# BICLab/Spike2Former

Measured on AMD Instinct MI355X. Metric: fwd+bwd images/sec, 512x512 T=4 ADE20K-150, higher is better.
Workload: dtype f32 (fp32-equivalent: bf16 hi+mid+lo split operands on bf16 MFMA, fp32 accumulate; spike maps stored as bf16, exact); 1 GPU; C2: 512x512 T=4 K=150 Meta-SpikeFormer [64, 128, 256, 360] + MaskFormer head, per-GPU batch 2; global_batch=2, parallelism=dp1, weights=random-init (name-seeded)

## Files before the change

spike2former_amd/csrc/pgemm.hip:

```cpp
#include "gemm_common.h"
#include <cstdlib>
#include <type_traits>

#pragma clang fp contract(fast)

namespace {

constexpr int PK = 32;
constexpr int PR = 64;
constexpr int PTERM = PR * PK;
constexpr int PBLOCK = 3 * PTERM;

typedef __attribute__((address_space(3))) void lds_void;
typedef const __attribute__((address_space(1))) void gbl_void;

__device__ __forceinline__ void dma16(const void* src, void* lds_dst) {
  __builtin_amdgcn_global_load_lds((gbl_void*)src, (lds_void*)lds_dst, 16, 0, 0);
}
template <int OFF>
__device__ __forceinline__ s16x4 lds_tr16_asm(unsigned byte_addr) {
  s16x4 r;
  asm volatile("ds_read_b64_tr_b16 %0, %1 offset:%2" : "=v"(r) : "v"(byte_addr), "n"(OFF));
  return r;
}
// ... 485 lines not shown
  f32x4 breg[NQ];
  auto fetch_b = [&](int tl) __attribute__((always_inline)) {
#pragma unroll
    for (int q = 0; q < NQ; ++q) {
      const int p = tid + q * T;
      const int k = p / (BN / 4), c4 = p % (BN / 4);
      const int kr = min((t_first + tl) * KC + k, Mo - 1);
      const int col = min(n0 + c4 * 4, N - 4);
      breg[q] = *reinterpret_cast<const f32x4*>(Gb + (int64_t)kr * N + col);
    }
  };
  auto stage_b = [&](int st) __attribute__((always_inline)) {
    unsigned short* Bs = reinterpret_cast<unsigned short*>(smem + st * STAGE + A_BYTES);
#pragma unroll
    for (int q = 0; q < NQ; ++q) {
      const int p = tid + q * T;
      const int k = p / (BN / 4), c4 = p % (BN / 4);
      const int off = k * BN + ((((c4 >> 3) ^ (k & 3)) << 5) | ((c4 & 7) << 2));
      unsigned int h0, m0_, l0_, h1, m1, l1;
      s2f_split3x2(breg[q].x, breg[q].y, h0, m0_, l0_);
      s2f_split3x2(breg[q].z, breg[q].w, h1, m1, l1);
      *reinterpret_cast<u32x2*>(Bs + off) = u32x2{h0, h1};
      *reinterpret_cast<u32x2*>(Bs + KC * BN + off) = u32x2{m0_, m1};
      *reinterpret_cast<u32x2*>(Bs + 2 * KC * BN + off) = u32x2{l0_, l1};
    }
  };

  f32x16 acc[MI][NJ];
#pragma unroll
  for (int i = 0; i < MI; ++i)
#pragma unroll
    for (int j = 0; j < NJ; ++j)
#pragma unroll
      for (int r = 0; r < 16; ++r) acc[i][j][r] = 0.f;

  const int kl = (lane & 15) >> 2, piece = lane & 3, hcol = (lane >> 4) & 1, kh = lane >> 5;
  int boff[NJ];
#pragma unroll
  for (int j = 0; j < NJ; ++j) boff[j] = (8 * kh + kl) * BN + (((wn * NJ + j) ^ kl) << 5) + 16 * hcol + 4 * piece;
  int aoff[MI][2];
#pragma unroll
  for (int i = 0; i < MI; ++i)
#pragma unroll
    for (int half = 0; half < 2; ++half) {
      const int row = 8 * kh + kl + 4 * half;
      const int c = (2 * hcol + (piece >> 1)) ^ ((2 * kh + half) & 3);
      aoff[i][half] = (wm * MI + i) * 512 + row * 32 + c * 8 + 4 * (piece & 1);
    }

  const unsigned smem_a = lds_addr(smem);
  auto compute = [&](int st) __attribute__((always_inline)) {
    union BF {
      bf16x8 v;
      s16x4 h[2];
    } bfrag[3][NJ], afrag[3][MI];
    const unsigned sb0 = smem_a + st * STAGE;
#pragma unroll
    for (int ks = 0; ks < KS; ++ks) {
      const unsigned sb = sb0 + ks * A_SLICE;
      const unsigned sbb = sb0 + ks * (16 * BN * 2);
#pragma unroll
      for (int j = 0; j < NJ; ++j) {
        const unsigned a = sbb + boff[j] * 2;
        bfrag[0][j].h[0] = lds_tr16_asm<A_BYTES>(a);
        bfrag[0][j].h[1] = lds_tr16_asm<A_BYTES + 4 * BN * 2>(a);
        bfrag[1][j].h[0] = lds_tr16_asm<A_BYTES + B_TERM>(a);
        bfrag[1][j].h[1] = lds_tr16_asm<A_BYTES + B_TERM + 4 * BN * 2>(a);
        bfrag[2][j].h[0] = lds_tr16_asm<A_BYTES + 2 * B_TERM>(a);
        bfrag[2][j].h[1] = lds_tr16_asm<A_BYTES + 2 * B_TERM + 4 * BN * 2>(a);
      }
#pragma unroll
      for (int i = 0; i < MI; ++i) {
        afrag[0][i].h[0] = lds_tr16_asm<0>(sb + aoff[i][0] * 2);
        afrag[0][i].h[1] = lds_tr16_asm<0>(sb + aoff[i][1] * 2);
      }
#pragma unroll
      for (int i = 0; i < MI; ++i) {
        afrag[1][i].h[0] = lds_tr16_asm<(BM / 32) * 1024>(sb + aoff[i][0] * 2);
        afrag[1][i].h[1] = lds_tr16_asm<(BM / 32) * 1024>(sb + aoff[i][1] * 2);
      }
#pragma unroll
      for (int i = 0; i < MI; ++i) {
        afrag[2][i].h[0] = lds_tr16_asm<2 * (BM / 32) * 1024>(sb + aoff[i][0] * 2);
        afrag[2][i].h[1] = lds_tr16_asm<2 * (BM / 32) * 1024>(sb + aoff[i][1] * 2);
      }
#pragma unroll
      for (int ta = 0; ta < 3; ++ta) {
        if (ta == 0) lds_wait<4 * MI>();
        if (ta == 1) lds_wait<2 * MI>();
        if (ta == 2) lds_wait<0>();
#pragma unroll
        for (int i = 0; i < MI; ++i)
#pragma unroll
          for (int tb = 0; tb < 3; ++tb)
            if (ta + tb < 3)
#pragma unroll
              for (int j = 0; j < NJ; ++j)
                mfma_bf16(acc[i][j], afrag[ta][i].v, bfrag[tb][j].v);
      }
    }
  };

  fetch_b(0);
  issue_a(0, 0);
  stage_b(0);
  if (nk > 1) fetch_b(1);
  for (int t = 0; t < nk; ++t) {
    const int st = t & 1;
    if (t + 1 < nk)
      wait_vm_and_barrier<NQ>();
    else
      wait_vm_and_barrier<0>();
    if (t + 1 < nk) {
      stage_b(st ^ 1);
      issue_a(t + 1, st ^ 1);
      if (t + 2 < nk) fetch_b(t + 2);
    }
    compute(st);
  }

  mfma_fence(acc);
  if constexpr (EPI == 3) {
    static_assert(2 * STAGE >= BM * BN * 4, "the output tile must fit the stages it is transposed through");
    epi_bn_lif<MI, NJ, WMW, WNW>(acc, ep, smem, m0, n0, Ki, N, b, wm, wn, lane, wave, dx_batch_stride);
    return;
  }
#pragma unroll
  for (int i = 0; i < MI; ++i)
#pragma unroll
    for (int j = 0; j < NJ; ++j) {
      const int col = n0 + (wn * NJ + j) * 32 + (lane & 31);
      float prev[16];
      if (BETA) {
#pragma unroll
        for (int r = 0; r < 16; ++r) {
          const int row = m0 + (wm * MI + i) * 32 + (r & 3) + 8 * (r >> 2) + 4 * (lane >> 5);
          prev[r] = Db[(int64_t)min(row, Ki - 1) * N + min(col, N - 1)];
        }
      }
#pragma unroll
      for (int r = 0; r < 16; ++r) {
        const int row = m0 + (wm * MI + i) * 32 + (r & 3) + 8 * (r >> 2) + 4 * (lane >> 5);
        if (row < Ki && col < N) {
          if (EPI == 2)
            atomicAdd(Db + (int64_t)row * N + col, acc[i][j][r]);
          else
            Db[(int64_t)row * N + col] = BETA ? acc[i][j][r] + beta * prev[r] : acc[i][j][r];
        }
      }
    }
  if constexpr (EPI == 0 && STATS)
    epi_row_partials<MI, NJ, WMW, WNW>(acc, part, n_tiles * (int)gridDim.y, reinterpret_cast<float*>(smem), m0, n0, Ki, N,
                                       b * n_tiles + nt, wm, wn, lane, tid);
}

template <int MI, int NJ, int WMW, int WNW, int NST>
__global__ __launch_bounds__(64 * WMW * WNW) void pg_tn_split_kernel(const unsigned short* __restrict__ Wp,
                                                                    const unsigned short* __restrict__ Gs, int64_t plane_stride,
                                                                    float* __restrict__ DX, int Mo, int Ki, int N, int KbW,
                                                                    int n_tiles, int m_tiles) {
  constexpr int BM = 32 * MI * WMW, BN = 32 * NJ * WNW, NW = WMW * WNW;
  constexpr int KC = 16;
  constexpr int A_BYTES = 3 * (BM / 32) * 1024, B_TERM = KC * BN * 2, B_BYTES = 3 * B_TERM, STAGE = A_BYTES + B_BYTES;
  constexpr int NA = 3 * (BM / 32), NAW = (NA + NW - 1) / NW;
  constexpr int NBT = B_TERM / 1024, NB = 3 * NBT, NBW = NB / NW;
  static_assert(NB % NW == 0 && BN == 128, "tile shape");
  constexpr int LPW = NAW + NBW;
  __shared__ __attribute__((aligned(1024))) unsigned char smem[NST * STAGE];

  const int tiles = n_tiles * m_tiles;
  int pid = blockIdx.x;
  if (tiles % 8 == 0) pid = (pid % 8) * (tiles / 8) + pid / 8;
  const int mt = pid % m_tiles, nt = pid / m_tiles;
  const int b = blockIdx.y;
  const int m0 = mt * BM, n0 = nt * BN;
  const unsigned short* Gb = Gs + (int64_t)b * Mo * N;
  float* Db = DX + (int64_t)b * Ki * N;
  const int tid = threadIdx.x, lane = tid & 63;
  const int wave = __builtin_amdgcn_readfirstlane((int)(tid >> 6));
  const int wm = wave / WNW, wn = wave % WNW;
  const int nk = (Mo + KC - 1) / KC;

  constexpr int CPRW = BN * 2 / 16;
  const int b_kl = lane / CPRW, b_pc = lane % CPRW;
  auto issue = [&](int t, int st) __attribute__((always_inline)) {
    unsigned char* sb = smem + st * STAGE;
    const int c0 = t * KC;
    const unsigned short* rows = Wp + (int64_t)(c0 / PR) * KbW * PBLOCK + (c0 % PR) * PK + lane * 8;
#pragma unroll
    for (int q = 0; q < NAW; ++q) {
      int idx = wave + q * NW;
      if (NA % NW != 0 && idx >= NA) idx -= NW;
      const int term = idx / (BM / 32), p = idx % (BM / 32);
      const int kb = min(m0 / PK + p, KbW - 1);
      dma16(rows + kb * PBLOCK + term * PTERM, sb + idx * 1024);
    }
#pragma unroll
    for (int q = 0; q < NBW; ++q) {
      const int idx = wave + q * NW;
      const int term = idx / NBT, r4 = idx % NBT;
      const int k = r4 * 4 + b_kl;
      const int lc = (((b_pc >> 2) ^ (k & 3)) << 2) | (b_pc & 3);
      const int kr = min(c0 + k, Mo - 1);
      const int col = min(n0 + lc * 8, N - 8);
      dma16(Gb + term * plane_stride + (int64_t)kr * N + col, sb + A_BYTES + idx * 1024);
    }
  };

  f32x16 acc[MI][NJ];
#pragma unroll
  for (int i = 0; i < MI; ++i)
#pragma unroll
    for (int j = 0; j < NJ; ++j)
#pragma unroll
      for (int r = 0; r < 16; ++r) acc[i][j][r] = 0.f;

  const int kl = (lane & 15) >> 2, piece = lane & 3, hcol = (lane >> 4) & 1, kh = lane >> 5;
  int boff[NJ];
#pragma unroll
  for (int j = 0; j < NJ; ++j) boff[j] = (8 * kh + kl) * BN + (((wn * NJ + j) ^ kl) << 5) + 16 * hcol + 4 * piece;
  int aoff[MI][2];
#pragma unroll
  for (int i = 0; i < MI; ++i)
#pragma unroll
    for (int half = 0; half < 2; ++half) {
      const int row = 8 * kh + kl + 4 * half;
      const int c = (2 * hcol + (piece >> 1)) ^ ((2 * kh + half) & 3);
      aoff[i][half] = (wm * MI + i) * 512 + row * 32 + c * 8 + 4 * (piece & 1);
    }

  const unsigned smem_a = lds_addr(smem);
  auto compute = [&](int st) __attribute__((always_inline)) {
    union BF {
      bf16x8 v;
      s16x4 h[2];
    } bfrag[3][NJ], afrag[3][MI];
    const unsigned sb = smem_a + st * STAGE;
#pragma unroll
    for (int j = 0; j < NJ; ++j) {
      const unsigned a = sb + boff[j] * 2;
      bfrag[0][j].h[0] = lds_tr16_asm<A_BYTES>(a);
      bfrag[0][j].h[1] = lds_tr16_asm<A_BYTES + 4 * BN * 2>(a);
      bfrag[1][j].h[0] = lds_tr16_asm<A_BYTES + B_TERM>(a);
      bfrag[1][j].h[1] = lds_tr16_asm<A_BYTES + B_TERM + 4 * BN * 2>(a);
      bfrag[2][j].h[0] = lds_tr16_asm<A_BYTES + 2 * B_TERM>(a);
      bfrag[2][j].h[1] = lds_tr16_asm<A_BYTES + 2 * B_TERM + 4 * BN * 2>(a);
    }
#pragma unroll
    for (int i = 0; i < MI; ++i) {
      afrag[0][i].h[0] = lds_tr16_asm<0>(sb + aoff[i][0] * 2);
      afrag[0][i].h[1] = lds_tr16_asm<0>(sb + aoff[i][1] * 2);
    }
#pragma unroll
    for (int i = 0; i < MI; ++i) {
      afrag[1][i].h[0] = lds_tr16_asm<(BM / 32) * 1024>(sb + aoff[i][0] * 2);
      afrag[1][i].h[1] = lds_tr16_asm<(BM / 32) * 1024>(sb + aoff[i][1] * 2);
    }
#pragma unroll
    for (int i = 0; i < MI; ++i) {
      afrag[2][i].h[0] = lds_tr16_asm<2 * (BM / 32) * 1024>(sb + aoff[i][0] * 2);
      afrag[2][i].h[1] = lds_tr16_asm<2 * (BM / 32) * 1024>(sb + aoff[i][1] * 2);
    }
#pragma unroll
    for (int ta = 0; ta < 3; ++ta) {
      if (ta == 0) lds_wait<4 * MI>();
      if (ta == 1) lds_wait<2 * MI>();
      if (ta == 2) lds_wait<0>();
#pragma unroll
      for (int i = 0; i < MI; ++i)
#pragma unroll
        for (int tb = 0; tb < 3; ++tb)
          if (ta + tb < 3)
#pragma unroll
            for (int j = 0; j < NJ; ++j)
              mfma_bf16(acc[i][j], afrag[ta][i].v, bfrag[tb][j].v);
    }
  };

#pragma unroll
  for (int s = 0; s < NST - 1; ++s)
    if (s < nk) issue(s, s);
  int st = 0, st_next = NST - 1;
  for (int t = 0; t < nk; ++t) {
    if (t + NST - 2 < nk)
      wait_vm_and_barrier<(NST - 2) * LPW>();
    else
      wait_vm_and_barrier<0>();
    if (t + NST - 1 < nk) issue(t + NST - 1, st_next);
    compute(st);
    st = st + 1 == NST ? 0 : st + 1;
    st_next = st_next + 1 == NST ? 0 : st_next + 1;
  }

  mfma_fence(acc);
#pragma unroll
  for (int i = 0; i < MI; ++i)
#pragma unroll
    for (int j = 0; j < NJ; ++j) {
      const int col = n0 + (wn * NJ + j) * 32 + (lane & 31);
#pragma unroll
      for (int r = 0; r < 16; ++r) {
        const int row = m0 + (wm * MI + i) * 32 + (r & 3) + 8 * (r >> 2) + 4 * (lane >> 5);
        if (row < Ki && col < N) Db[(int64_t)row * N + col] = acc[i][j][r];
      }
    }
}
// ... 459 lines not shown
               (const float*)nullptr, (float*)nullptr, M, N, K, Kb, n_tiles, m_tiles, Conv3{0, 0, 0}, (float*)nullptr, ep);
  }
  return s2f_check_launch("s2f_gemm_bn_lif_fwd");
}

extern "C" int s2f_conv3x3_bn_lif_fwd(const uint16_t* w_pack, const uint16_t* X, const float* conv_bias, const float* running_mean,
                                      const float* running_var, const float* gamma, const float* beta, float eps,
                                      const float* residual, float* u_out, const float* v_in, void* y_bf16, float* v_out,
                                      uint64_t* stats, int batch, int M, int C, int H, int W, float vth, int D, void* stream) {
  S2F_REQUIRE(w_pack && X && running_mean && running_var && gamma && beta, S2F_EINVAL, "s2f_conv3x3_bn_lif_fwd: null pointer");
  S2F_REQUIRE(u_out || y_bf16, S2F_EINVAL, "s2f_conv3x3_bn_lif_fwd: neither u_out nor y requested");
  S2F_REQUIRE(batch > 0 && batch < 65536 && M > 0 && C > 0 && C % 32 == 0 && H > 0 && W >= 4 && (W & 3) == 0, S2F_EINVAL,
              "s2f_conv3x3_bn_lif_fwd: need C %% 32 == 0 and W %% 4 == 0 (C=%d, W=%d)", C, W);
  S2F_REQUIRE(!y_bf16 || s2f_bf16_spikes_exact(D), S2F_EINVAL, "s2f_conv3x3_bn_lif_fwd: bf16 spikes need D a power of two <= 128");
  S2F_REQUIRE(s2f_aligned16(w_pack) && (reinterpret_cast<uintptr_t>(X) & 7u) == 0, S2F_EALIGN,
              "s2f_conv3x3_bn_lif_fwd: pack 16-byte, activation 8-byte aligned");
  const int N = H * W, K = 9 * C, Kb = K / PK, n_tiles = (N + 127) / 128;
  BnLifEpi ep{conv_bias, running_mean, running_var, gamma, beta, residual, u_out, v_in, v_out,
              reinterpret_cast<unsigned short*>(y_bf16), reinterpret_cast<unsigned long long*>(stats), eps, vth, (float)D,
              1.0f / (float)D};
  hipStream_t s = (hipStream_t)stream;
  const Conv3 geo{H, W, C};
  static const char* small_env = getenv("S2F_PG_CONV_SMALL");
  const bool small_ok = !(small_env && small_env[0] == '0');
  const bool narrow = small_ok && M > 64 && (int64_t)n_tiles * batch * ((M + 127) / 128) <= 256;
#define S2F_PGCE(MI, NJ, WMW, WNW)                                                                                        \
  do {                                                                                                                   \
    const int m_tiles = (M + 32 * MI * WMW - 1) / (32 * MI * WMW);                                                       \
    if (small_ok && (Kb & 1) == 0 && Kb >= 4 && (int64_t)n_tiles * m_tiles * batch <= 512)                               \
      S2F_LAUNCH(true, true, (pg_conv_kernel<MI, NJ, WMW, WNW, 1, true, false, 1, 2>), dim3(n_tiles * m_tiles, batch),    \
                 dim3(64 * WMW * WNW), 0, s, w_pack, X, (const float*)nullptr, (float*)nullptr, M, N, K, Kb, n_tiles, m_tiles, \
                 geo, (float*)nullptr, ep);                                                                              \
    else                                                                                                                 \
      S2F_LAUNCH(true, true, (pg_conv_kernel<MI, NJ, WMW, WNW, 1, true, false, 1>), dim3(n_tiles * m_tiles, batch),       \
                 dim3(64 * WMW * WNW), 0, s, w_pack, X, (const float*)nullptr, (float*)nullptr, M, N, K, Kb, n_tiles, m_tiles, \
                 geo, (float*)nullptr, ep);                                                                              \
  } while (0)
  if (M <= 32)
    S2F_PGCE(1, 1, 1, 4);
  else if (M <= 64 || narrow)
    S2F_PGCE(1, 2, 2, 2);
  else
    S2F_PGCE(1, 2, 4, 2);
#undef S2F_PGCE
  return s2f_check_launch("s2f_conv3x3_bn_lif_fwd");
}

extern "C" int s2f_pgemm_dx_split(const uint16_t* w_pack, const uint16_t* G_split, int64_t plane_stride, float* DX, int batch,
                                  int Mo, int Ki, int N, int cfg, void* stream) {
  S2F_REQUIRE(w_pack && G_split && DX, S2F_EINVAL, "s2f_pgemm_dx_split: null pointer");
  S2F_REQUIRE(batch > 0 && batch < 65536 && Mo > 0 && Ki > 0 && N >= 8 && (N & 7) == 0, S2F_EINVAL,
              "s2f_pgemm_dx_split: bad sizes (N=%d must be a positive multiple of 8)", N);
  S2F_REQUIRE(s2f_aligned16(w_pack) && s2f_aligned16(G_split) && s2f_aligned16(DX) && (plane_stride & 7) == 0, S2F_EALIGN,
              "s2f_pgemm_dx_split: pointers / plane stride must keep 16-byte alignment");
  hipStream_t s = (hipStream_t)stream;
  const int KbW = (Ki + PK - 1) / PK;
  const int n_tiles = (N + 127) / 128;
  static const char* force = getenv("S2F_PG_DXS_CFG");
  int c = cfg > 0 ? cfg : (force ? atoi(force) : 0);
  if (c <= 0) c = (Ki > 64 && (int64_t)n_tiles * batch * ((Ki + 127) / 128) >= 512) ? 1 : 2;
#define S2F_PGS(MI, NJ, WMW, WNW, NSTV)                                                                                 \
  do {                                                                                                                 \
    const int m_tiles = (Ki + 32 * MI * WMW - 1) / (32 * MI * WMW);                                                    \
    S2F_LAUNCH(true, true, (pg_tn_split_kernel<MI, NJ, WMW, WNW, NSTV>), dim3(n_tiles * m_tiles, batch),                \
               dim3(64 * WMW * WNW), 0, s, w_pack, G_split, plane_stride, DX, Mo, Ki, N, KbW, n_tiles, m_tiles);        \
  } while (0)
  switch (c) {
    case 1: S2F_PGS(2, 2, 2, 2, 3); break;
    case 2: S2F_PGS(1, 2, 2, 2, 3); break;
    case 3: S2F_PGS(2, 2, 2, 2, 2); break;
    case 4: S2F_PGS(1, 2, 2, 2, 2); break;
    default: S2F_REQUIRE(false, S2F_EINVAL, "s2f_pgemm_dx_split: unknown cfg %d", c);
  }
#undef S2F_PGS
  return s2f_check_launch("s2f_pgemm_dx_split");
}

static int conv_launch(const char* who, const uint16_t* w_pack, const void* X, bool x_fp32, const float* bias, float* Y, int batch,
                       int M, int C, int H, int W, int cfg, void* stream, float* part = nullptr) {
  S2F_REQUIRE(w_pack && X && Y, S2F_EINVAL, "%s: null pointer", who);
  S2F_REQUIRE(!part || (!bias && (reinterpret_cast<uintptr_t>(part) & 7u) == 0), S2F_EINVAL,
              "%s: the statistics are those of the product without a bias; partials 8-byte aligned", who);
  S2F_REQUIRE(batch > 0 && batch < 65536 && M > 0 && C > 0 && C % 32 == 0 && H > 0 && W >= 4 && (W & 3) == 0, S2F_EINVAL,
              "%s: need C %% 32 == 0 and W %% 4 == 0 (C=%d, W=%d)", who, C, W);
  S2F_REQUIRE((int64_t)C * 9 < (1 << 30) && (int64_t)H * W < (1 << 30), S2F_EINVAL, "%s: too large", who);
  S2F_REQUIRE(s2f_aligned16(w_pack) && s2f_aligned16(Y) && (reinterpret_cast<uintptr_t>(X) & (x_fp32 ? 15u : 7u)) == 0, S2F_EALIGN,
              "%s: pack / output 16-byte, activation 8-byte (bf16) or 16-byte (fp32) aligned", who);
  hipStream_t s = (hipStream_t)stream;
  const int N = H * W, K = 9 * C, Kb = K / PK;
  const int n_tiles = (N + 127) / 128;
  static const char* force = getenv("S2F_PG_CONV_CFG");
  int c = cfg > 0 ? cfg : (force ? atoi(force) : 0);
  if (c <= 0) c = M <= 32 ? 3 : M <= 64 ? 2 : 4;
  static const char* small_env = getenv("S2F_PG_CONV_SMALL");
  const bool small_ok = !(small_env && small_env[0] == '0');
  if (cfg <= 0 && !force && small_ok && c == 4 && (int64_t)n_tiles * batch * ((M + 127) / 128) <= 256) c = 2;
  const bool g2 = small_ok && !x_fp32 &&
                  nn_super_steps(Kb, (int64_t)n_tiles * batch * ((M + (c == 4 || c == 1 ? 127 : c == 2 ? 63 : 31)) / (c == 4 || c == 1 ? 128 : c == 2 ? 64 : 32)));
  const Conv3 geo{H, W, C};
#define S2F_PGC(MI, NJ, WMW, WNW)                                                                                         \
  do {                                                                                                                   \
    const int m_tiles = (M + 32 * MI * WMW - 1) / (32 * MI * WMW);                                                       \
    if (x_fp32)                                                                                                          \
      S2F_LAUNCH(true, true, (pg_conv_kernel<MI, NJ, WMW, WNW, 3>), dim3(n_tiles * m_tiles, batch), dim3(64 * WMW * WNW), 0, s, \
                 w_pack, X, bias, Y, M, N, K, Kb, n_tiles, m_tiles, geo, part, BnLifEpi{});                                           \
    else if (part && g2)                                                                                                 \
      S2F_LAUNCH(true, true, (pg_conv_kernel<MI, NJ, WMW, WNW, 1, true, true, 0, 2>), dim3(n_tiles * m_tiles, batch),     \
                 dim3(64 * WMW * WNW), 0, s, w_pack, X, bias, Y, M, N, K, Kb, n_tiles, m_tiles, geo, part, BnLifEpi{});               \
    else if (g2)                                                                                                         \
      S2F_LAUNCH(true, true, (pg_conv_kernel<MI, NJ, WMW, WNW, 1, true, false, 0, 2>), dim3(n_tiles * m_tiles, batch),    \
                 dim3(64 * WMW * WNW), 0, s, w_pack, X, bias, Y, M, N, K, Kb, n_tiles, m_tiles, geo, part, BnLifEpi{});               \
    else if (part)                                                                                                       \
      S2F_LAUNCH(true, true, (pg_conv_kernel<MI, NJ, WMW, WNW, 1, true, true>), dim3(n_tiles * m_tiles, batch),           \
                 dim3(64 * WMW * WNW), 0, s, w_pack, X, bias, Y, M, N, K, Kb, n_tiles, m_tiles, geo, part, BnLifEpi{});               \
    else                                                                                                                 \
      S2F_LAUNCH(true, true, (pg_conv_kernel<MI, NJ, WMW, WNW, 1>), dim3(n_tiles * m_tiles, batch), dim3(64 * WMW * WNW), 0, s, \
                 w_pack, X, bias, Y, M, N, K, Kb, n_tiles, m_tiles, geo, part, BnLifEpi{});                                           \
  } while (0)
  switch (c) {
    case 1: S2F_PGC(2, 2, 2, 2); break;
    case 2: S2F_PGC(1, 2, 2, 2); break;
    case 3: S2F_PGC(1, 1, 1, 4); break;
    case 4: S2F_PGC(1, 2, 4, 2); break;
    default: S2F_REQUIRE(false, S2F_EINVAL, "%s: unknown cfg %d", who, c);
  }
#undef S2F_PGC
  return s2f_check_launch(who);
}

extern "C" int s2f_pgemm_conv3x3_bf16(const uint16_t* w_pack, const uint16_t* X, const float* bias, float* Y, int batch, int M, int C,
                                      int H, int W, int cfg, void* stream) {
  return conv_launch("s2f_pgemm_conv3x3_bf16", w_pack, X, false, bias, Y, batch, M, C, H, W, cfg, stream);
}

extern "C" int s2f_pgemm_conv3x3_bf16_stats(const uint16_t* w_pack, const uint16_t* X, float* Y, float* bn_partials, int batch,
                                            int M, int C, int H, int W, void* stream) {
  S2F_REQUIRE(bn_partials, S2F_EINVAL, "s2f_pgemm_conv3x3_bf16_stats: null partials");
  return conv_launch("s2f_pgemm_conv3x3_bf16_stats", w_pack, X, false, nullptr, Y, batch, M, C, H, W, 0, stream, bn_partials);
}

extern "C" int s2f_pgemm_conv3x3_f32(const uint16_t* w_pack, const float* X, float* Y, int batch, int M, int C, int H, int W,
                                     int cfg, void* stream) {
  return conv_launch("s2f_pgemm_conv3x3_f32", w_pack, X, true, nullptr, Y, batch, M, C, H, W, cfg, stream);
}

extern "C" int s2f_pack_bf16x3(const float* src, uint16_t* dst, int M, int K, int mode, int C, void* stream) {
  S2F_REQUIRE(src && dst && M > 0 && K > 0 && mode >= 0 && mode <= 3, S2F_EINVAL, "s2f_pack_bf16x3: bad arguments");
  S2F_REQUIRE((mode != 1 && mode != 2) || C > 0, S2F_EINVAL, "s2f_pack_bf16x3: conv modes need C");
  const int64_t wgs = (int64_t)((M + PR - 1) / PR) * ((K + PK - 1) / PK) * (PTERM / 1024);
  hipLaunchKernelGGL(pack_one_kernel, dim3((unsigned)wgs), dim3(256), 0, (hipStream_t)stream, src, dst, M, K, mode, C);
  return s2f_check_launch("s2f_pack_bf16x3");
}

static int pgemm_dx_impl(const uint16_t* w_pack, const float* G, int64_t g_batch_stride, float* DX, int64_t dx_batch_stride,
                         int batch, int Mo, int Ki, int N, float beta, int cfg, float* part, void* stream) {
  if (g_batch_stride == 0) g_batch_stride = (int64_t)Mo * N;
  S2F_REQUIRE(!part || (beta == 0.f && (reinterpret_cast<uintptr_t>(part) & 7u) == 0), S2F_EINVAL,
              "s2f_pgemm_dx_f32_stats: plain-store form only; partials 8-byte aligned");
  if (dx_batch_stride == 0) dx_batch_stride = (int64_t)Ki * N;
  S2F_REQUIRE((g_batch_stride & 3) == 0 && (dx_batch_stride & 3) == 0, S2F_EALIGN, "s2f_pgemm_dx_f32: batch strides must keep 16-byte alignment");
  S2F_REQUIRE(w_pack && G && DX, S2F_EINVAL, "s2f_pgemm_dx_f32: null pointer");
  S2F_REQUIRE(batch > 0 && batch < 65536 && Mo > 0 && Ki > 0 && N >= 4 && (N & 3) == 0, S2F_EINVAL,
              "s2f_pgemm_dx_f32: bad sizes (N=%d must be a positive multiple of 4)", N);
  S2F_REQUIRE(s2f_aligned16(w_pack) && s2f_aligned16(G) && s2f_aligned16(DX), S2F_EALIGN,
              "s2f_pgemm_dx_f32: pointers must be 16-byte aligned");
  hipStream_t s = (hipStream_t)stream;
  const int KbW = (Ki + PK - 1) / PK;
  const int n_tiles = (N + 127) / 128;
  static const char* force = getenv("S2F_PG_DX_CFG");
  int c = cfg > 0 ? cfg : (force ? atoi(force) : 0);
  static const char* t3e = getenv("S2F_PG_DX_T3");
  const int64_t t3 = t3e ? atoll(t3e) : 192;
  if (c <= 0) c = Ki <= 32 ? 5 : (Ki > 64 && (int64_t)n_tiles * batch * ((Ki + 127) / 128) >= t3) ? 3 : (beta == 0.f ? 7 : 4);
  static const char* ks4 = getenv("S2F_PG_DX_KS4");
  if (c == 7 && !(ks4 && ks4[0] == '0') && Mo >= 128 && (int64_t)n_tiles * batch * ((Ki + 63) / 64) <= 512) c = 10;
  int zsplit = 1;
  {
    const int64_t wgs = (int64_t)n_tiles * batch * ((Ki + 63) / 64);
    const int steps = (Mo + 15) / 16;
    while ((beta == 0.f || beta == 1.f) && !part && wgs * zsplit < 128 && steps / (zsplit * 2) >= 16) zsplit *= 2;
  }
  if (zsplit > 1) {
    S2F_REQUIRE(dx_batch_stride == (int64_t)Ki * N, S2F_EINVAL, "s2f_pgemm_dx_f32: the split form needs a dense DX");
    if (beta == 0.f && s2f_zero_async(DX, sizeof(float) * (size_t)batch * Ki * N, s) != S2F_OK)
      return s2f_check_launch("s2f_pgemm_dx_f32 zero");
    c = 4;
  }
#define S2F_PGD(MI, NJ, WMW, WNW)                                                                                       \
  do {                                                                                                                 \
    const int m_tiles = (Ki + 32 * MI * WMW - 1) / (32 * MI * WMW);                                                    \
    const dim3 grid(n_tiles * m_tiles, batch, zsplit);                                                                 \
    if (zsplit > 1)                                                                                                    \
      S2F_LAUNCH(true, true, (pg_tn_f32_kernel<MI, NJ, WMW, WNW, 2>), grid, dim3(64 * WMW * WNW), 0, s, w_pack, G, DX,  \
                 Mo, Ki, N, KbW, n_tiles, m_tiles, beta, g_batch_stride, dx_batch_stride, (float*)nullptr, TnGroups{}, BnLifEpi{});          \
    else if (beta != 0.f)                                                                                              \
      S2F_LAUNCH(true, true, (pg_tn_f32_kernel<MI, NJ, WMW, WNW, 1>), grid, dim3(64 * WMW * WNW), 0, s, w_pack, G, DX,   \
                 Mo, Ki, N, KbW, n_tiles, m_tiles, beta, g_batch_stride, dx_batch_stride, (float*)nullptr, TnGroups{}, BnLifEpi{});          \
    else if (part)                                                                                                     \
      S2F_LAUNCH(true, true, (pg_tn_f32_kernel<MI, NJ, WMW, WNW, 0, 1, true>), grid, dim3(64 * WMW * WNW), 0, s, w_pack, \
                 G, DX, Mo, Ki, N, KbW, n_tiles, m_tiles, beta, g_batch_stride, dx_batch_stride, part, TnGroups{}, BnLifEpi{});         \
    else                                                                                                               \
      S2F_LAUNCH(true, true, (pg_tn_f32_kernel<MI, NJ, WMW, WNW, 0>), grid, dim3(64 * WMW * WNW), 0, s, w_pack, G, DX,   \
                 Mo, Ki, N, KbW, n_tiles, m_tiles, beta, g_batch_stride, dx_batch_stride, part, TnGroups{}, BnLifEpi{});                \
  } while (0)
  switch (c) {
    case 1: S2F_PGD(2, 2, 2, 2); break;
    case 2: S2F_PGD(1, 2, 2, 2); break;
    case 3: S2F_PGD(1, 2, 4, 2); break;
    case 4: S2F_PGD(1, 1, 2, 4); break;
    case 5: S2F_PGD(1, 1, 1, 4); break;
#define S2F_PGD2(MI, NJ, WMW, WNW) S2F_PGD3(MI, NJ, WMW, WNW, 2)
#define S2F_PGD3(MI, NJ, WMW, WNW, KSV)                                                                                 \
  do {                                                                                                                 \
    S2F_REQUIRE(zsplit == 1 && beta == 0.f, S2F_EINVAL, "s2f_pgemm_dx_f32: cfg %d is the plain store form", c);           \
    const int m_tiles = (Ki + 32 * MI * WMW - 1) / (32 * MI * WMW);                                                    \
    if (part)                                                                                                          \
      S2F_LAUNCH(true, true, (pg_tn_f32_kernel<MI, NJ, WMW, WNW, 0, KSV, true>), dim3(n_tiles * m_tiles, batch, 1),      \
                 dim3(64 * WMW * WNW), 0, s, w_pack, G, DX, Mo, Ki, N, KbW, n_tiles, m_tiles, beta, g_batch_stride,      \
                 dx_batch_stride, part, TnGroups{}, BnLifEpi{});                                                                       \
    else                                                                                                               \
      S2F_LAUNCH(true, true, (pg_tn_f32_kernel<MI, NJ, WMW, WNW, 0, KSV>), dim3(n_tiles * m_tiles, batch, 1),            \
                 dim3(64 * WMW * WNW), 0, s, w_pack, G, DX, Mo, Ki, N, KbW, n_tiles, m_tiles, beta, g_batch_stride,      \
                 dx_batch_stride, part, TnGroups{}, BnLifEpi{});                                                                       \
  } while (0)
    case 7: S2F_PGD2(1, 1, 2, 4); break;
    case 8: S2F_PGD2(1, 2, 2, 2); break;
    case 9: S2F_PGD2(1, 2, 4, 2); break;
    case 10: S2F_PGD3(1, 1, 2, 4, 4); break;
#undef S2F_PGD3
#undef S2F_PGD2
    default: S2F_REQUIRE(false, S2F_EINVAL, "s2f_pgemm_dx_f32: unknown cfg %d", c);
  }
#undef S2F_PGD
  return s2f_check_launch("s2f_pgemm_dx_f32");
}

extern "C" int s2f_pgemm_dx_f32(const uint16_t* w_pack, const float* G, int64_t g_batch_stride, float* DX,
                                int64_t dx_batch_stride, int batch, int Mo, int Ki, int N, float beta, int cfg, void* stream) {
  return pgemm_dx_impl(w_pack, G, g_batch_stride, DX, dx_batch_stride, batch, Mo, Ki, N, beta, cfg, nullptr, stream);
}

extern "C" int s2f_pgemm_dx_f32_stats(const uint16_t* w_pack, const float* G, int64_t g_batch_stride, float* DX,
                                      int64_t dx_batch_stride, float* bn_partials, int batch, int Mo, int Ki, int N,
                                      void* stream) {
  S2F_REQUIRE(bn_partials, S2F_EINVAL, "s2f_pgemm_dx_f32_stats: null partials");
  return pgemm_dx_impl(w_pack, G, g_batch_stride, DX, dx_batch_stride, batch, Mo, Ki, N, 0.f, 0, bn_partials, stream);
}

extern "C" int s2f_dense_gemm_bn_lif_fwd(const uint16_t* const* w_packs, int groups, const float* X, int64_t x_batch_stride,
                                         int64_t x_group_stride, const float* conv_bias, const float* running_mean,
                                         const float* running_var, const float* gamma, const float* beta, float eps,
                                         const float* residual, float* u_out, void* y_bf16, uint64_t* stats, int batch, int K,
                                         int M, int N, float vth, int D, void* stream) {
  S2F_REQUIRE(w_packs && X && running_mean && running_var && gamma && beta && groups >= 1 && groups <= 4, S2F_EINVAL,
              "s2f_dense_gemm_bn_lif_fwd: null pointer / 1..4 groups");
  S2F_REQUIRE(u_out || y_bf16, S2F_EINVAL, "s2f_dense_gemm_bn_lif_fwd: neither u_out nor y requested");
  S2F_REQUIRE(batch > 0 && batch < 65536 && M > 0 && K > 0 && N >= 4 && (N & 3) == 0, S2F_EINVAL,
              "s2f_dense_gemm_bn_lif_fwd: bad sizes (N=%d must be a positive multiple of 4)", N);
  S2F_REQUIRE(!y_bf16 || s2f_bf16_spikes_exact(D), S2F_EINVAL, "s2f_dense_gemm_bn_lif_fwd: bf16 spikes need D a power of two <= 128");
  S2F_REQUIRE((x_batch_stride & 3) == 0 && (x_group_stride & 3) == 0 && s2f_aligned16(X) && (!residual || s2f_aligned16(residual)) &&
                  (!u_out || s2f_aligned16(u_out)) && (reinterpret_cast<uintptr_t>(y_bf16) & 7u) == 0,
              S2F_EALIGN, "s2f_dense_gemm_bn_lif_fwd: strides / pointers must keep 16-byte alignment");
  TnGroups grp{};
  for (int g = 0; g < groups; ++g) {
    S2F_REQUIRE(w_packs[g] && s2f_aligned16(w_packs[g]), S2F_EINVAL, "s2f_dense_gemm_bn_lif_fwd: null / unaligned pack %d", g);
    grp.wp[g] = w_packs[g];
  }
  grp.g_stride = x_group_stride;
  grp.dx_stride = (int64_t)M * N;
  BnLifEpi ep{conv_bias, running_mean, running_var, gamma, beta, residual, u_out, nullptr, nullptr,
              reinterpret_cast<unsigned short*>(y_bf16), reinterpret_cast<unsigned long long*>(stats), eps, vth, (float)D,
              1.0f / (float)D};
  hipStream_t s = (hipStream_t)stream;
  const int KbW = (M + PK - 1) / PK, n_tiles = (N + 127) / 128;
  const int64_t out_bs = (int64_t)groups * M * N;
  const bool wide = M > 64 && (int64_t)n_tiles * batch * ((M + 127) / 128) >= 192;
#define S2F_PGE(MI, NJ, WMW, WNW, KSV)                                                                                   \
  do {                                                                                                                  \
    const int m_tiles = (M + 32 * MI * WMW - 1) / (32 * MI * WMW);                                                      \
    S2F_LAUNCH(true, true, (pg_tn_f32_kernel<MI, NJ, WMW, WNW, 3, KSV, false, true>), dim3(n_tiles * m_tiles, batch, groups),    \
               dim3(64 * WMW * WNW), 0, s, grp.wp[0], X, (float*)nullptr, K, M, N, KbW, n_tiles, m_tiles, 0.f, x_batch_stride,  \
               out_bs, (float*)nullptr, grp, ep);                                                                       \
  } while (0)
  if (M <= 32)
    S2F_PGE(1, 1, 1, 4, 1);
  else if (wide)
    S2F_PGE(1, 2, 4, 2, 2);
  else if (K >= 128 && (int64_t)n_tiles * batch * ((M + 63) / 64) * groups <= 512)
    S2F_PGE(1, 1, 2, 4, 4);
  else
    S2F_PGE(1, 1, 2, 4, 2);
#undef S2F_PGE
  return s2f_check_launch("s2f_dense_gemm_bn_lif_fwd");
}

extern "C" int s2f_pgemm_dx_f32_grouped(const uint16_t* const* w_packs, int groups, const float* G, int64_t g_batch_stride,
                                        int64_t g_group_stride, float* DX, int64_t dx_batch_stride, int64_t dx_group_stride,
                                        float* bn_partials, int64_t partials_group_stride, int batch, int Mo, int Ki, int N,
                                        void* stream) {
  S2F_REQUIRE(w_packs && G && DX && groups >= 1 && groups <= 4, S2F_EINVAL, "s2f_pgemm_dx_f32_grouped: null pointer / 1..4 groups");
  S2F_REQUIRE(batch > 0 && batch < 65536 && Mo > 0 && Ki > 0 && N >= 4 && (N & 3) == 0, S2F_EINVAL,
              "s2f_pgemm_dx_f32_grouped: bad sizes (N=%d must be a positive multiple of 4)", N);
  S2F_REQUIRE((g_batch_stride & 3) == 0 && (dx_batch_stride & 3) == 0 && (g_group_stride & 3) == 0 && (dx_group_stride & 3) == 0 &&
                  s2f_aligned16(G) && s2f_aligned16(DX) && (reinterpret_cast<uintptr_t>(bn_partials) & 7u) == 0,
              S2F_EALIGN, "s2f_pgemm_dx_f32_grouped: strides / pointers must keep 16-byte alignment");
  TnGroups grp{};
  for (int g = 0; g < groups; ++g) {
    S2F_REQUIRE(w_packs[g] && s2f_aligned16(w_packs[g]), S2F_EINVAL, "s2f_pgemm_dx_f32_grouped: null / unaligned pack %d", g);
    grp.wp[g] = w_packs[g];
  }
  grp.g_stride = g_group_stride;
  grp.dx_stride = dx_group_stride;
  grp.part_stride = partials_group_stride;
  hipStream_t s = (hipStream_t)stream;
  const int KbW = (Ki + PK - 1) / PK, n_tiles = (N + 127) / 128;
  const bool wide = Ki > 64 && (int64_t)n_tiles * batch * ((Ki + 127) / 128) >= 192;
#define S2F_PGG(MI, NJ, WMW, WNW, KSV)                                                                                   \
  do {                                                                                                                  \
    const int m_tiles = (Ki + 32 * MI * WMW - 1) / (32 * MI * WMW);                                                     \
    const dim3 grid(n_tiles * m_tiles, batch, groups);                                                                  \
    if (bn_partials)                                                                                                    \
      S2F_LAUNCH(true, true, (pg_tn_f32_kernel<MI, NJ, WMW, WNW, 0, KSV, true, true>), grid, dim3(64 * WMW * WNW), 0, s,  \
                 grp.wp[0], G, DX, Mo, Ki, N, KbW, n_tiles, m_tiles, 0.f, g_batch_stride, dx_batch_stride, bn_partials, grp, BnLifEpi{}); \
    else                                                                                                                \
      S2F_LAUNCH(true, true, (pg_tn_f32_kernel<MI, NJ, WMW, WNW, 0, KSV, false, true>), grid, dim3(64 * WMW * WNW), 0, s, \
                 grp.wp[0], G, DX, Mo, Ki, N, KbW, n_tiles, m_tiles, 0.f, g_batch_stride, dx_batch_stride, bn_partials, grp, BnLifEpi{}); \
  } while (0)
  if (Ki <= 32)
    S2F_PGG(1, 1, 1, 4, 1);
  else if (wide)
    S2F_PGG(1, 2, 4, 2, 1);
  else
    S2F_PGG(1, 1, 2, 4, 2);
#undef S2F_PGG
  return s2f_check_launch("s2f_pgemm_dx_f32_grouped");
}
```

Baseline: 54.53 images/s.

## Add register-fed dX GEMM kernel that splits G into bf16x3 in registers

Adds a new transposed-GEMM kernel for the dX backward pass. It loads the fp32 gradient G straight from global memory into registers, splits it into bf16 hi/mid/lo fragments there, and streams only the packed weights through a double-buffered LDS ring using buffer loads. A heuristic routes small-N or narrow-Ki, large-N shapes (plain and grouped) to this kernel. The goal is to avoid staging G through LDS and to fit skinny shapes better, at the cost of higher register pressure and uncoalesced per-row global loads of G.

```diff
diff --git a/spike2former_amd/csrc/pgemm.hip b/spike2former_amd/csrc/pgemm.hip
--- a/spike2former_amd/csrc/pgemm.hip
+++ b/spike2former_amd/csrc/pgemm.hip
@@ -661,6 +661,163 @@
   if constexpr (EPI == 0 && STATS)
     epi_row_partials<MI, NJ, WMW, WNW>(acc, part, n_tiles * (int)gridDim.y, reinterpret_cast<float*>(smem), m0, n0, Ki, N,
                                        b * n_tiles + nt, wm, wn, lane, tid);
+}
+
+__device__ __forceinline__ void dma16_buf(const void* base, unsigned bytes, unsigned off, void* lds_dst) {
+  const __amdgpu_buffer_rsrc_t r = __builtin_amdgcn_make_buffer_rsrc(const_cast<void*>(base), 0, bytes, 0x00020000);
+  __builtin_amdgcn_raw_ptr_buffer_load_lds(r, (lds_void*)lds_dst, 16, off, 0, 0, 0);
+}
+
+template <int MI, int NJ, int WNW, int CH, bool GROUPED = false>
+__global__ __launch_bounds__(64 * WNW) void pg_tn_rf_kernel(const unsigned short* __restrict__ Wp, const float* __restrict__ G,
+                                                           float* __restrict__ DX, int Mo, int Ki, int N, int KbW, int n_tiles,
+                                                           int m_tiles, int64_t g_batch_stride, int64_t dx_batch_stride,
+                                                           TnGroups grp) {
+  if constexpr (GROUPED) {
+    const int g = blockIdx.z;
+    Wp = grp.wp[g];
+    G += g * grp.g_stride;
+    DX += g * grp.dx_stride;
+  }
+  constexpr int BM = 32 * MI, NW = WNW;
+  constexpr int SLICE = 3 * MI * 1024;
+  constexpr int CHUNK = CH * SLICE;
+  constexpr int NC = CH * 3 * MI;
+  constexpr int D = 2;
+  static_assert(CH % D == 0 && 4 * MI <= 15, "ring slot of a slice must be a compile-time constant; lgkmcnt is 4 bits");
+  __shared__ __attribute__((aligned(1024))) unsigned char smem[2 * CHUNK];
+
+  const int tiles = n_tiles * m_tiles;
+  int pid = blockIdx.x;
+  if (tiles % 8 == 0) pid = (pid % 8) * (tiles / 8) + pid / 8;
+  const int mt = pid % m_tiles, nt = pid / m_tiles;
+  const int b = blockIdx.y;
+  const int m0 = mt * BM, n0 = nt * (32 * NJ * WNW);
+  const float* Gb = G + (int64_t)b * g_batch_stride;
+  float* Db = DX + (int64_t)b * dx_batch_stride;
+  const int lane = threadIdx.x & 63;
+  const int wave = __builtin_amdgcn_readfirstlane((int)(threadIdx.x >> 6));
+  const int nsl = (Mo + 15) / 16, nch = (nsl + CH - 1) / CH;
+  const unsigned pack_bytes = (unsigned)((int64_t)((Mo + PR - 1) / PR) * KbW * PBLOCK * 2);
+
+  auto issue_chunk = [&](int c) __attribute__((always_inline)) {
+    unsigned char* sb = smem + (c & 1) * CHUNK;
+#pragma unroll
+    for (int q = 0; q < (NC + NW - 1) / NW; ++q) {
+      const int idx = wave + q * NW;
+      if (NC % NW != 0 && idx >= NC) break;
+      const int s = idx / (3 * MI), term = (idx / MI) % 3, p = idx % MI;
+      const int c0 = (c * CH + s) * 16;
+      const int kb = min(m0 / PK + p, KbW - 1);
+      const int64_t e = ((int64_t)(c0 / PR) * KbW + kb) * PBLOCK + term * PTERM + (c0 % PR) * PK;
+      dma16_buf(Wp, pack_bytes, c0 < Mo ? (unsigned)(e * 2) + lane * 16 : 0xfffffff0u, sb + idx * 1024);
+    }
+  };
+  float raw[D][NJ][8];
+  const int kh = lane >> 5;
+  int gcol[NJ];
+#pragma unroll
+  for (int j = 0; j < NJ; ++j) gcol[j] = min(n0 + (wave * NJ + j) * 32 + (lane & 31), N - 1);
+  auto load_slice = [&](int sl, float (&r)[NJ][8]) __attribute__((always_inline)) {
+#pragma unroll
+    for (int e = 0; e < 8; ++e) {
+      const int kr = min(sl * 16 + 8 * kh + e, Mo - 1);
+#pragma unroll
+      for (int j = 0; j < NJ; ++j) r[j][e] = Gb[(int64_t)kr * N + gcol[j]];
+    }
+  };
+
+  f32x16 acc[MI][NJ];
+#pragma unroll
+  for (int i = 0; i < MI; ++i)
+#pragma unroll
+    for (int j = 0; j < NJ; ++j)
+#pragma unroll
+      for (int r = 0; r < 16; ++r) acc[i][j][r] = 0.f;
+
+  const int kl = (lane & 15) >> 2, piece = lane & 3, hcol = (lane >> 4) & 1;
+  int aoff[MI][2];
+#pragma unroll
+  for (int i = 0; i < MI; ++i)
+#pragma unroll
+    for (int half = 0; half < 2; ++half) {
+      const int row = 8 * kh + kl + 4 * half;
+      const int c = (2 * hcol + (piece >> 1)) ^ ((2 * kh + half) & 3);
+      aoff[i][half] = (i * 512 + row * 32 + c * 8 + 4 * (piece & 1)) * 2;
+    }
+  const unsigned smem_a = lds_addr(smem);
+
+  auto run_chunk = [&](int c, bool next) __attribute__((always_inline)) {
+    wait_vm_and_barrier<D * NJ * 8>();
+    if (next) issue_chunk(c + 1);
+    const unsigned sb = smem_a + (c & 1) * CHUNK;
+#pragma unroll
+    for (int s = 0; s < CH; ++s) {
+      const int sl = c * CH + s;
+      union BF {
+        bf16x8 v;
+        unsigned u[4];
+        s16x4 h[2];
+      } bfrag[3][NJ], afrag[3][MI];
+#pragma unroll
+      for (int j = 0; j < NJ; ++j)
+#pragma unroll
+        for (int p = 0; p < 4; ++p)
+          s2f_split3x2(raw[s % D][j][2 * p], raw[s % D][j][2 * p + 1], bfrag[0][j].u[p], bfrag[1][j].u[p], bfrag[2][j].u[p]);
+      load_slice(sl + D, raw[s % D]);
+      const unsigned sa = sb + s * SLICE;
+#pragma unroll
+      for (int i = 0; i < MI; ++i) {
+        afrag[0][i].h[0] = lds_tr16_asm<0>(sa + aoff[i][0]);
+        afrag[0][i].h[1] = lds_tr16_asm<0>(sa + aoff[i][1]);
+      }
+#pragma unroll
+      for (int i = 0; i < MI; ++i) {
+        afrag[1][i].h[0] = lds_tr16_asm<MI * 1024>(sa + aoff[i][0]);
+        afrag[1][i].h[1] = lds_tr16_asm<MI * 1024>(sa + aoff[i][1]);
+      }
+#pragma unroll
+      for (int i = 0; i < MI; ++i) {
+        afrag[2][i].h[0] = lds_tr16_asm<2 * MI * 1024>(sa + aoff[i][0]);
+        afrag[2][i].h[1] = lds_tr16_asm<2 * MI * 1024>(sa + aoff[i][1]);
+      }
+#pragma unroll
+      for (int t = 0; t < 3; ++t)
+#pragma unroll
+        for (int j = 0; j < NJ; ++j) asm volatile("" : "+v"(bfrag[t][j].v));
+#pragma unroll
+      for (int ta = 0; ta < 3; ++ta) {
+        if (ta == 0) asm volatile("s_waitcnt lgkmcnt(%0)\n\ts_nop 1" ::"n"(4 * MI) : "memory");
+        if (ta == 1) lds_wait<2 * MI>();
+        if (ta == 2) lds_wait<0>();
+#pragma unroll
+        for (int i = 0; i < MI; ++i)
+#pragma unroll
+          for (int tb = 0; tb < 3; ++tb)
+            if (ta + tb < 3)
+#pragma unroll
+              for (int j = 0; j < NJ; ++j) mfma_bf16(acc[i][j], afrag[ta][i].v, bfrag[tb][j].v);
+      }
+    }
+  };
+  issue_chunk(0);
+#pragma unroll
+  for (int d = 0; d < D; ++d) load_slice(d, raw[d]);
+  for (int c = 0; c + 1 < nch; ++c) run_chunk(c, true);
+  run_chunk(nch - 1, false);
+
+  mfma_fence(acc);
+#pragma unroll
+  for (int i = 0; i < MI; ++i)
+#pragma unroll
+    for (int j = 0; j < NJ; ++j) {
+      const int col = n0 + (wave * NJ + j) * 32 + (lane & 31);
+#pragma unroll
+      for (int r = 0; r < 16; ++r) {
+        const int row = m0 + i * 32 + (r & 3) + 8 * (r >> 2) + 4 * kh;
+        if (row < Ki && col < N) Db[(int64_t)row * N + col] = acc[i][j][r];
+      }
+    }
 }
 
 template <int MI, int NJ, int WMW, int WNW, int NST>
@@ -1426,6 +1583,15 @@
   return s2f_check_launch("s2f_pack_bf16x3");
 }
 
+static int pgemm_dx_rf_cfg(int old, int batch, int Mo, int Ki, int N) {
+  static const char* ab = getenv("S2F_PG_DX_RF");
+  if (ab && ab[0] == '0') return old;
+  (void)batch;
+  if (N <= 128 && Ki <= 256 && Mo <= 256) return 11;
+  if (Ki <= 64 && Mo >= 64 && N >= 16384) return Ki <= 32 && Mo >= 256 ? 11 : 12;
+  return old;
+}
+
 static int pgemm_dx_impl(const uint16_t* w_pack, const float* G, int64_t g_batch_stride, float* DX, int64_t dx_batch_stride,
                          int batch, int Mo, int Ki, int N, float beta, int cfg, float* part, void* stream) {
   if (g_batch_stride == 0) g_batch_stride = (int64_t)Mo * N;
@@ -1452,8 +1618,10 @@
   {
     const int64_t wgs = (int64_t)n_tiles * batch * ((Ki + 63) / 64);
     const int steps = (Mo + 15) / 16;
-    while ((beta == 0.f || beta == 1.f) && !part && wgs * zsplit < 128 && steps / (zsplit * 2) >= 16) zsplit *= 2;
-  }
+    while (c < 11 && (beta == 0.f || beta == 1.f) && !part && wgs * zsplit < 128 && steps / (zsplit * 2) >= 16) zsplit *= 2;
+  }
+  if (cfg <= 0 && !force && zsplit == 1 && beta == 0.f && !part && s2f_pack_elems(Mo, Ki) * 2 < (int64_t(1) << 31))
+    c = pgemm_dx_rf_cfg(c, batch, Mo, Ki, N);
   if (zsplit > 1) {
     S2F_REQUIRE(dx_batch_stride == (int64_t)Ki * N, S2F_EINVAL, "s2f_pgemm_dx_f32: the split form needs a dense DX");
     if (beta == 0.f && s2f_zero_async(DX, sizeof(float) * (size_t)batch * Ki * N, s) != S2F_OK)
@@ -1503,6 +1671,19 @@
     case 10: S2F_PGD3(1, 1, 2, 4, 4); break;
 #undef S2F_PGD3
 #undef S2F_PGD2
+#define S2F_PGR(MI, NJ, WNW, CH)                                                                                         \
+  do {                                                                                                                 \
+    S2F_REQUIRE(zsplit == 1 && beta == 0.f && !part, S2F_EINVAL, "s2f_pgemm_dx_f32: cfg %d is the plain store form", c);  \
+    S2F_REQUIRE(s2f_pack_elems(Mo, Ki) * 2 < (int64_t(1) << 31), S2F_EINVAL, "s2f_pgemm_dx_f32: cfg %d: pack over 2 GiB", c); \
+    static_assert(32 * NJ * WNW == 128, "n_tiles counts 128-column tiles");                                             \
+    const int m_tiles = (Ki + 32 * MI - 1) / (32 * MI);                                                                \
+    S2F_LAUNCH(true, true, (pg_tn_rf_kernel<MI, NJ, WNW, CH>), dim3(n_tiles * m_tiles, batch, 1), dim3(64 * WNW), 0, s, \
+               w_pack, G, DX, Mo, Ki, N, KbW, n_tiles, m_tiles, g_batch_stride, dx_batch_stride, TnGroups{});          \
+  } while (0)
+    case 11: S2F_PGR(1, 1, 4, 8); break;
+    case 12: S2F_PGR(2, 1, 4, 4); break;
+    case 13: S2F_PGR(1, 2, 2, 8); break;
+#undef S2F_PGR
     default: S2F_REQUIRE(false, S2F_EINVAL, "s2f_pgemm_dx_f32: unknown cfg %d", c);
   }
 #undef S2F_PGD
@@ -1600,12 +1781,26 @@
       S2F_LAUNCH(true, true, (pg_tn_f32_kernel<MI, NJ, WMW, WNW, 0, KSV, false, true>), grid, dim3(64 * WMW * WNW), 0, s, \
                  grp.wp[0], G, DX, Mo, Ki, N, KbW, n_tiles, m_tiles, 0.f, g_batch_stride, dx_batch_stride, bn_partials, grp, BnLifEpi{}); \
   } while (0)
-  if (Ki <= 32)
+#define S2F_PGGR(MI, NJ, WNW, CH)                                                                                        \
+  do {                                                                                                                  \
+    const int m_tiles = (Ki + 32 * MI - 1) / (32 * MI);                                                                 \
+    S2F_LAUNCH(true, true, (pg_tn_rf_kernel<MI, NJ, WNW, CH, true>), dim3(n_tiles * m_tiles, batch, groups), dim3(64 * WNW), \
+               0, s, grp.wp[0], G, DX, Mo, Ki, N, KbW, n_tiles, m_tiles, g_batch_stride, dx_batch_stride, grp);        \
+  } while (0)
+  const int old = Ki <= 32 ? 5 : wide ? 3 : 7;
+  const int rf = bn_partials || old == 5 || s2f_pack_elems(Mo, Ki) * 2 >= (int64_t(1) << 31)
+                     ? old : pgemm_dx_rf_cfg(old, batch * groups, Mo, Ki, N);
+  if (rf == 11)
+    S2F_PGGR(1, 1, 4, 8);
+  else if (rf == 12)
+    S2F_PGGR(2, 1, 4, 4);
+  else if (Ki <= 32)
     S2F_PGG(1, 1, 1, 4, 1);
   else if (wide)
     S2F_PGG(1, 2, 4, 2, 1);
   else
     S2F_PGG(1, 1, 2, 4, 2);
+#undef S2F_PGGR
 #undef S2F_PGG
   return s2f_check_launch("s2f_pgemm_dx_f32_grouped");
 }
```

Result: no change. 54.53 images/s (median of 3 runs) (+0.0%).
